# johannes-graeter/mono_lidar_depth

Measured on AMD Instinct MI355X. Metric: feature-depth associations/sec, higher is better.
Workload: dtype f64; 1 GPU; BASELINE config 2: 64x2048 cloud x 2000 features/frame, C0 parameters, 1024 HBM-resident frames/step/GPU; frame_slots_per_launch=1024, features_per_frame=2000, points_per_frame=131072, contexts=2, sequences=1, parallelism=sequence-per-gpu x1

## Files before the change

mono_lidar_depth_amd/csrc/mld_api.hip:

```cpp
#include <hip/hip_runtime.h>

#include <algorithm>

#include <cmath>
#include <cstdio>
#include <cstdlib>
#include <condition_variable>
#include <cstring>
#include <ctime>
#include <functional>
#include <limits>
#include <mutex>
#include <string>
#include <thread>
#include <vector>

#include "../../include/mld.h"
#include "mld_device.h"
#include "mld_kernels.hip"
#include "mld_ransac.hip"

using namespace mld;

namespace {
// ... 31 lines not shown

struct TimedLaunch {
    hipEvent_t e0, e1;
    int which;
};

}

struct FrameHelper {
    std::thread th;
    std::mutex m;
    std::condition_variable cv;
    std::function<int(std::string&)> job;
    bool pending = false, quit = false;
    int rc = 0;
    std::string err;
    void run() {
        std::unique_lock<std::mutex> lk(m);
        for (;;) {
            cv.wait(lk, [&] { return pending || quit; });
            if (quit) return;
            std::function<int(std::string&)> j = std::move(job);
            lk.unlock();
            std::string e;
            const int r = j(e);
            lk.lock();
            rc = r;
            err = std::move(e);
            pending = false;
            cv.notify_all();
        }
    }
    void submit(std::function<int(std::string&)> j) {
        {
            std::lock_guard<std::mutex> lk(m);
            job = std::move(j);
            pending = true;
        }
        cv.notify_all();
    }
    int wait(std::string& e) {
        std::unique_lock<std::mutex> lk(m);
        cv.wait(lk, [&] { return !pending; });
        e = err;
        return rc;
    }
    void stop() {
        {
            std::lock_guard<std::mutex> lk(m);
            quit = true;
        }
        cv.notify_all();
        if (th.joinable()) th.join();
    }
};

struct ProjShare {
    hipStream_t stream = nullptr;
    int refs = 0;
};

struct mld_ctx {
    mld_params P{};
    mld_camera cam{};
    Calib calib{};
    int device = 0;
    hipStream_t stream = nullptr;
    bool own_stream = true;
    std::vector<Slot> slots;
    SlotDesc* d_slots = nullptr;
    unsigned char* dummy = nullptr;
    int32_t* queue_counts = nullptr;
    uint32_t* map_slab = nullptr;
    size_t map_stride = 0;
    int32_t* queue_slab = nullptr;
    uint32_t* bitmaps = nullptr;
    size_t bitmap_words = 0;
    std::vector<SlotDesc> h_descs;
    std::vector<SlotDesc> desc_stage;
    size_t lds_bytes = 0;
    size_t lds_fused = 0;
    size_t lds_classify = 0;
    bool classify_staged = true;
    int bm_ncol = 0, bm_ncolp = 0;
    bool force_thread_path = false;
    size_t proj_lds = 0;
    std::string err;
    int32_t* rs_flags = nullptr;
    int32_t* rs_cand = nullptr;
    int32_t* rs_block = nullptr;
    size_t rs_cap = 0;
    int32_t* rs_M = nullptr;
    int32_t* rs_S = nullptr;
    int32_t* rs_sample = nullptr;
    float* rs_sp = nullptr;
    int32_t* rs_counts = nullptr;
    size_t rs_counts_cap = 0;
    int32_t* rs_inl = nullptr;
    ransac::Result* rs_res = nullptr;
    unsigned char* sem_img = nullptr;
    size_t sem_img_cap = 0;
    float* sem_coeffs = nullptr;
    unsigned char* sem_groups = nullptr;
    size_t sem_groups_cap = 0;
    ransac::SemResult* sem_res = nullptr;
    double* trk_uv_cur = nullptr;
    double* trk_uv_last = nullptr;
    double* trk_depth_cur = nullptr;
    double* trk_depth_last = nullptr;
    int32_t* trk_type_cur = nullptr;
    int32_t* trk_type_last = nullptr;
    int32_t* trk_rank = nullptr;
    long long* trk_n_new = nullptr;
    size_t trk_cap = 0;
    unsigned char* trkb = nullptr;
    size_t trkb_cap = 0;
    int trkb_seqs = 0;
    TrkSeq* trkb_desc = nullptr;
    std::vector<TrkSeq> trkb_host;
    SlotDesc* d_sub = nullptr;
    int32_t* sub_counts = nullptr;
    size_t sub_cap = 0;
    std::vector<SlotDesc> h_sub;
    unsigned char* trk_stage = nullptr;
    size_t trk_stage_cap = 0;
    unsigned char* fr_host = nullptr;
    unsigned char* fr_dev = nullptr;
    size_t fr_cap = 0;
    unsigned char* fr_host_dev = nullptr;
    bool fr_zero_copy = true;
    bool fr_helper_on = true;
    hipEvent_t fr_ev[5] = {nullptr, nullptr, nullptr, nullptr, nullptr};
    double fr_us[10] = {0, 0, 0, 0, 0, 0, 0, 0, 0, 0};
    uint32_t* rsb_masks = nullptr;
    size_t rsb_mask_words = 0;
    PlaneDev* rsb_planes = nullptr;
    uint32_t* rsb_seeds = nullptr;
    hipStream_t side = nullptr;
    hipEvent_t side_done = nullptr, side_start = nullptr;
    FrameHelper* helper = nullptr;
    hipEvent_t order_ev = nullptr;
    mld_ctx* release_waiter = nullptr;
    mld_ctx* waiting_on = nullptr;
    bool order_wait_pending = false;
    uint32_t* cls_done = nullptr;
    uint32_t cls_target = 0;
    const uint32_t* gate_counter = nullptr;
    uint32_t gate_target = 0;
    bool gate_mode = true;
    Calib* d_calib = nullptr;
    Calib calib_uploaded[2]{};
    mld_ctx* gate_src = nullptr;
    mld_ctx* gate_waiter = nullptr;
    hipStream_t proj_stream = nullptr;
    struct ProjShare* proj_share = nullptr;
    hipEvent_t proj_fork = nullptr, proj_join = nullptr;
    size_t lds_fused_pad = 0;
    int queue_probe_tries = 0;
    int queue_shared_with_live = 0;
    int shared_arg = 0;
    int fused_blocks_per_cu = 8;
    size_t lds_per_cu = 0;
    bool timing = false;
    std::vector<TimedLaunch> timed;
    std::vector<hipEvent_t> event_pool;
    static constexpr int kUpGens = 16;
// ... 124 lines not shown
            for (int k = 0; k < 3; k++) {
                ri += (long double)c.Tinv[4 * i + k] * (long double)T[4 * k + 3];
                mi += fabsl((long double)c.Tinv[4 * i + k]) * fabsl((long double)T[4 * k + 3]);
            }
            lin = std::max(lin, rl);
            mlin = std::max(mlin, ml);
            cst = std::max(cst, fabsl(ri));
            mcst = std::max(mcst, mi);
        }
        const long double u64 = 1.1102230246251565e-16L;
        const long double el = lin + 64.0L * u64 * mlin, ec = cst + 64.0L * u64 * mcst;
        const float inf = std::numeric_limits<float>::infinity();
        c.far_elin = (std::isfinite((double)el) && el < 1e30L) ? (float)((double)el * 1.000001) : inf;
        c.far_econst = (std::isfinite((double)ec) && ec < 1e30L) ? (float)((double)ec * 1.000001) : inf;
        if (!(c.far_elin > 0.f)) c.far_elin = 1e-37f;
    }
    c.W = ctx->cam.width;
    c.H = ctx->cam.height;
    c.bmStride = (ctx->cam.height + 16 + 3) / 4 * 4;
    c.halfX1 = (double)P.pixelarea_search_witdh * 0.5 * (double)1.0f;
    c.halfY1 = (double)P.pixelarea_search_height * 0.5 * (double)1.0f;
    c.halfX2 = (double)P.pixelarea_search_witdh * 0.5 * (double)2.0f;
    c.halfY2 = (double)P.pixelarea_search_height * 0.5 * (double)1.5f;
    int cap = window_cells(c.halfX1, c.halfY1);
    if (P.do_use_ransac_plane) cap = std::max(cap, window_cells(c.halfX2, c.halfY2));
    cap = (cap + 1) & ~1;
    c.cap = cap;
    c.binW = P.histogram_segmentation_bin_witdh;
    c.minCount = P.histogram_segmentation_min_pointcount;
    c.countMin = (unsigned)P.radiusSearch_count_min;
    c.useHist = P.do_use_histogram_segmentation;
    c.thrG_en = P.treshold_depth_enabled;
    c.thrG_mode = P.treshold_depth_mode;
    c.thrG_min = (double)P.treshold_depth_min;
    c.thrG_max = (double)P.treshold_depth_max;
    c.thrL_en = P.treshold_depth_local_enabled;
    c.thrL_mode = P.treshold_depth_local_mode;
    c.thrL_type = P.treshold_depth_local_valuetype;
    c.thrL_val = P.treshold_depth_local_value;
    c.useTriMax = P.do_use_triangle_size_maximation;
    c.checkPlanar = P.do_check_triangleplanar_condition;
    c.planarThr = P.triangleplanar_crossnorm_treshold;
    c.orthThr = P.viewray_plane_orthoganality_treshold;
    c.cutBehind = P.do_use_cut_behind_camera;
    c.useRoad = P.do_use_ransac_plane;
    c.roadMode = P.plane_estimator_use_triangle_maximation ? 1 : 0;
    c.roadDistThr = P.ransac_plane_point_distance_treshold;
    c.roadDistThrF = (float)c.roadDistThr;
    c.padf2_ = 0.f;
    c.zxMinRel = P.plane_estimator_z_x_min_relation;
    c.usePCA = P.do_use_PCA;
    c.pcaAbsMin = P.pca_treshold_3_abs_min;
    c.pcaRelMax = P.pca_treshold_3_2_rel_max;
    c.pcaRelMin = P.pca_treshold_2_1_rel_min;
    ctx->lds_bytes = (size_t)cap * (3 * sizeof(double) + 2 * sizeof(int));
    c.threadPath = 1;
    c.xcdAware = 1;
    c.sortClasses = 4;
    c.k1max = 32;
    c.kMain = 24;
    c.kTotal = 40;
#ifdef MLD_AB_SWITCHES
    if (const char* e = std::getenv("MLD_FORCE_WAVE_PATH")) c.threadPath = (e[0] == '1') ? 0 : 1;
    if (const char* e = std::getenv("MLD_NO_XCD")) c.xcdAware = (e[0] == '1') ? 0 : 1;
    if (const char* e = std::getenv("MLD_SORT_CLASSES")) c.sortClasses = (e[0] == '4') ? 4 : 1;
    if (const char* e = std::getenv("MLD_FORCE_THREAD_PATH")) ctx->force_thread_path = e[0] == '1';
    if (const char* e = std::getenv("MLD_PROJ_LDS")) ctx->proj_lds = (size_t)std::atoll(e);
    if (const char* e = std::getenv("MLD_GATE")) ctx->gate_mode = e[0] != '0';
    if (const char* e = std::getenv("MLD_FRAME_COPY")) ctx->fr_zero_copy = e[0] != '1';
    if (const char* e = std::getenv("MLD_FRAME_HELPER")) ctx->fr_helper_on = e[0] != '0';
    if (const char* e = std::getenv("MLD_K1MAX")) c.k1max = std::min(std::max(std::atoi(e), 8), kK1MaxLimit);
    if (const char* e = std::getenv("MLD_KMAIN")) c.kMain = std::min(std::max(std::atoi(e), 8), c.k1max);
    if (std::getenv("MLD_K1MAX") || std::getenv("MLD_KMAIN")) c.kTotal = c.k1max + c.kMain;
    if (const char* e = std::getenv("MLD_KTOTAL")) c.kTotal = std::min(std::max(std::atoi(e), c.k1max), c.k1max + c.kMain);
#endif
    ctx->lds_fused = (size_t)c.kTotal * kWave * sizeof(uint32_t);
    ctx->bm_ncol = (ctx->cam.width + 31) / 32 + 1;
    ctx->bm_ncolp = ctx->bm_ncol | 1;
    const size_t cls_fixed = (size_t)(kClsBuckets + kClsThreads / kWave + 4) * sizeof(int);
    const size_t cls_bitmap = (size_t)c.bmStride * (size_t)ctx->bm_ncolp * sizeof(uint32_t);
    ctx->classify_staged = cls_fixed + cls_bitmap <= 128 * 1024;
#ifdef MLD_AB_SWITCHES
    if (const char* e = std::getenv("MLD_CLASSIFY_STAGED")) ctx->classify_staged = ctx->classify_staged && e[0] != '0';
#endif
    ctx->lds_classify = cls_fixed + (ctx->classify_staged ? cls_bitmap : 0);
}

hipStream_t projection_fork(mld_ctx* ctx, int& rc) {
    rc = MLD_OK;
    if (!ctx->proj_stream) return ctx->stream;
    hipError_t e = hipEventRecord(ctx->proj_fork, ctx->stream);
    if (e == hipSuccess) e = hipStreamWaitEvent(ctx->proj_stream, ctx->proj_fork, 0);
    if (e != hipSuccess) {
        ctx->err = std::string("projection stream (fork): ") + hipGetErrorString(e);
        rc = MLD_ERR_HIP;
    }
    return ctx->proj_stream;
}
int projection_join(mld_ctx* ctx) {
    if (!ctx->proj_stream) return MLD_OK;
    HIP_TRY(ctx, hipEventRecord(ctx->proj_join, ctx->proj_stream));
    HIP_TRY(ctx, hipStreamWaitEvent(ctx->stream, ctx->proj_join, 0));
    return MLD_OK;
}
struct ProjectionScope {
    mld_ctx* ctx;
    bool open = true;
    explicit ProjectionScope(mld_ctx* c) : ctx(c) {}
    int finish() {
        open = false;
        return projection_join(ctx);
    }
    ~ProjectionScope() {
        if (open && ctx->proj_stream) {
            const std::string keep = ctx->err;
            (void)projection_join(ctx);
            ctx->err = keep;
        }
    }
};

int enable_rs_batch_lds(mld_ctx* ctx, size_t lds) {
    static size_t enabled[64] = {};
    static std::mutex mtx;
    std::lock_guard<std::mutex> lk(mtx);
    size_t& cur = enabled[ctx->device & 63];
    if (lds <= cur) return MLD_OK;
    HIP_TRY(ctx, hipFuncSetAttribute(reinterpret_cast<const void*>(ransac::k_rs_batch),
                                     hipFuncAttributeMaxDynamicSharedMemorySize, (int)lds));
    cur = lds;
    return MLD_OK;
}

int check_slot(mld_ctx* ctx, int slot) {
    if (!ctx) return MLD_ERR_INVALID_ARG;
    if (slot < 0 || slot >= (int)ctx->slots.size()) return fail(ctx, MLD_ERR_INVALID_ARG, "slot out of range");
    return MLD_OK;
}

int bind_device(mld_ctx* ctx) {
    HIP_TRY(ctx, hipSetDevice(ctx->device));
    return MLD_OK;
}

template <typename T>
int grow(mld_ctx* ctx, T*& ptr, size_t& cap, size_t need) {
    if (need <= cap && ptr) return MLD_OK;
    if (ptr) {
        HIP_TRY(ctx, hipStreamSynchronize(ctx->stream));
        HIP_TRY(ctx, hipFree(ptr));
        ptr = nullptr;
    }
    size_t n = need < 1 ? 1 : need;
    HIP_TRY(ctx, hipMalloc(reinterpret_cast<void**>(&ptr), n * sizeof(T)));
    cap = n;
    return MLD_OK;
}

hipEvent_t get_event(mld_ctx* ctx) {
    if (!ctx->event_pool.empty()) {
        hipEvent_t e = ctx->event_pool.back();
        ctx->event_pool.pop_back();
        return e;
    }
    hipEvent_t e = nullptr;
    (void)hipEventCreate(&e);
// ... 88 lines not shown
    bool aligned = true;
    for (int i = slot; i < slot + (single ? 1 : n_slots); i++)
        aligned = aligned && (((uintptr_t)ctx->slots[i].d.cloud) & 15) == 0;
    const uint32_t ps_magic = per_slot > 1 ? (uint32_t)(((1ull << 32) + (uint64_t)per_slot - 1) / (uint64_t)per_slot) : 0u;
    if (ctx->order_wait_pending) {
        ctx->order_wait_pending = false;
        if (ctx->gate_counter) {
            hipLaunchKernelGGL(mld::k_gate, dim3(1), dim3(kWave), 0, st, ctx->gate_counter, ctx->gate_target, 100000);
            ctx->gate_counter = nullptr;
            if (ctx->gate_src && ctx->gate_src->gate_waiter == ctx) ctx->gate_src->gate_waiter = nullptr;
            ctx->gate_src = nullptr;
        } else {
            HIP_TRY(ctx, hipStreamWaitEvent(st, ctx->order_ev, 0));
        }
    }
    ScopedTimer tm(ctx, 0, st);
    if (single) {
        auto kp = aligned ? mld::k_project_scatter<true, true> : mld::k_project_scatter<false, true>;
        hipLaunchKernelGGL(kp, dim3(per_slot), dim3(kProjThreads), 0, st, ctx->d_slots, ctx->slots[slot].d, ctx->calib, 1,
                           per_slot, ps_magic, 0u);
    } else {
        auto kp = aligned ? mld::k_project_scatter<true, false> : mld::k_project_scatter<false, false>;
        hipLaunchKernelGGL(kp, dim3((unsigned)per_slot * n_slots), dim3(kProjThreads), ctx->proj_lds, st, ctx->d_slots + slot,
                           SlotDesc{}, ctx->calib, n_slots, per_slot, ps_magic, common_tag(ctx, n_slots, slot));
    }
    HIP_TRY(ctx, hipGetLastError());
    return MLD_OK;
}

int ensure_queues(mld_ctx* ctx, Slot& s, int64_t F) {
    if ((size_t)F <= s.road_cap) return MLD_OK;
    HIP_TRY(ctx, hipStreamSynchronize(ctx->stream));
    if (!s.queues_in_slab) {
        if (s.d.ovf_queue) HIP_TRY(ctx, hipFree(s.d.ovf_queue));
        if (s.d.live_queue) HIP_TRY(ctx, hipFree(s.d.live_queue));
    }
    s.queues_in_slab = false;
    s.d.live_queue = nullptr;
    s.d.ovf_queue = nullptr;
    HIP_TRY(ctx, hipMalloc((void**)&s.d.ovf_queue, (size_t)F * 2 * sizeof(int32_t)));
    HIP_TRY(ctx, hipMalloc((void**)&s.d.live_queue, (size_t)F * sizeof(int32_t)));
    s.road_cap = (size_t)F;
    return MLD_OK;
}

int upload_descs(mld_ctx* ctx, int n_slots, hipStream_t st = nullptr, int first = 0, bool tags_in_descs = false);

int upload_small(mld_ctx* ctx, void* dst, const void* src, size_t bytes, hipStream_t st) {
    static_assert(sizeof(SlotDesc) % 4 == 0 && sizeof(TrkSeq) % 4 == 0 && sizeof(Calib) % 4 == 0, "k_upload moves 32-bit words");
    if (!bytes) return MLD_OK;
    if (bytes % 4) return fail(ctx, MLD_ERR_INVALID_ARG, "upload_small: size not a multiple of 4");
    if (bytes > ctx->up_gen_bytes) return fail(ctx, MLD_ERR_CAPACITY, "upload_small: table larger than the context's upload ring");
    const int g = ctx->up_next;
    if (ctx->up_busy[g]) HIP_TRY(ctx, hipEventSynchronize(ctx->up_ev[g]));
    if (!ctx->up_ev[g]) HIP_TRY(ctx, hipEventCreateWithFlags(&ctx->up_ev[g], hipEventDisableTiming));
    unsigned char* stage = ctx->up_base + (size_t)g * ctx->up_gen_bytes;
    std::memcpy(stage, src, bytes);
    const int words = (int)(bytes / 4);
    hipLaunchKernelGGL(mld::k_upload, dim3((unsigned)((words + 255) / 256)), dim3(256), 0, st, reinterpret_cast<uint32_t*>(dst),
                       reinterpret_cast<const uint32_t*>(stage), words);
    HIP_TRY(ctx, hipGetLastError());
    HIP_TRY(ctx, hipEventRecord(ctx->up_ev[g], st));
    ctx->up_busy[g] = true;
    ctx->up_next = (g + 1) % mld_ctx::kUpGens;
    return MLD_OK;
}

int launch_features(mld_ctx* ctx, int n_slots, int64_t max_F, bool single, int slot, const Calib* override_calib = nullptr,
                    const SlotDesc* group_descs = nullptr) {
    if (max_F <= 0) return MLD_OK;
    const SlotDesc* const descs = group_descs ? group_descs : ctx->d_slots;
    Calib calib = override_calib ? *override_calib : ctx->calib;
    const bool few = single && max_F <= 16384 && !ctx->force_thread_path;
    if (few) calib.threadPath = 0;
    const int per_slot = (int)((max_F + kWave - 1) / kWave);
    const uint32_t tag_all = (single || group_descs) ? 0u : common_tag(ctx, n_slots);
    const SlotDesc one = single ? ctx->slots[slot].d : SlotDesc{};
    const int use_single = single ? 1 : 0, ns = single ? 1 : n_slots;
    if (few) {
    } else {
        ScopedTimer ts(ctx, 5);
        auto kc = ctx->classify_staged ? mld::k_classify<true, kClsThreads, kClsKeep>
                                       : mld::k_classify<false, kClsThreads, kClsKeep>;
        const bool gate = ctx->gate_mode && ctx->release_waiter && !single;
        if (gate && !ctx->cls_done) {
            HIP_TRY(ctx, hipMalloc((void**)&ctx->cls_done, sizeof(uint32_t)));
            HIP_TRY(ctx, hipMemsetAsync(ctx->cls_done, 0, sizeof(uint32_t), ctx->stream));
        }
        hipLaunchKernelGGL(kc, dim3((unsigned)ns), dim3(kClsThreads), ctx->lds_classify, ctx->stream, descs, one,
                           use_single, calib, ctx->bm_ncol, ctx->bm_ncolp, gate ? ctx->cls_done : (uint32_t*)nullptr);
        if (gate) {
            mld_ctx* w = ctx->release_waiter;
            ctx->release_waiter = nullptr;
            w->waiting_on = nullptr;
            ctx->cls_target += (uint32_t)ns;
            if (w->gate_src && w->gate_src != ctx && w->gate_src->gate_waiter == w) w->gate_src->gate_waiter = nullptr;
            if (ctx->gate_waiter && ctx->gate_waiter != w) {
                ctx->gate_waiter->gate_counter = nullptr;
                ctx->gate_waiter->order_wait_pending = false;
                ctx->gate_waiter->gate_src = nullptr;
            }
            w->gate_counter = ctx->cls_done;
            w->gate_target = ctx->cls_target;
            w->order_wait_pending = true;
            w->gate_src = ctx;
            ctx->gate_waiter = w;
        }
    }
    if (ctx->release_waiter) {
        mld_ctx* w = ctx->release_waiter;
        ctx->release_waiter = nullptr;
        w->waiting_on = nullptr;
        HIP_TRY(ctx, hipEventRecord(w->order_ev, ctx->stream));
        if (w->gate_src && w->gate_src->gate_waiter == w) w->gate_src->gate_waiter = nullptr;
        w->gate_src = nullptr;
        w->gate_counter = nullptr;
        w->order_wait_pending = true;
    }
    int rc_up = MLD_OK;
    const Calib* d_calib = ctx->d_calib;
    {
        Calib want = calib;
        want.threadPath = ctx->calib.threadPath;
        const int which = std::memcmp(&want, &ctx->calib, sizeof(Calib)) == 0 ? 0 : 1;
        if (std::memcmp(&want, &ctx->calib_uploaded[which], sizeof(Calib)) != 0) {
            int rc_c = upload_small(ctx, ctx->d_calib + which, &want, sizeof(Calib), ctx->stream);
            if (rc_c) return rc_c;
            ctx->calib_uploaded[which] = want;
        }
        d_calib = ctx->d_calib + which;
    }
    if (calib.threadPath) {
        ScopedTimer tm(ctx, 1);
        int dense = (calib.k1max > 32 || calib.kMain > 24) ? ((ctx->shared_arg & 1) ? 1 : 2) : 0;
#ifdef MLD_AB_SWITCHES
        if (const char* e = std::getenv("MLD_FORCE_DENSE")) dense = std::min(std::max(std::atoi(e), 0), 2);
#endif
        auto kf = dense == 2 ? (calib.roadMode ? mld::k_feature_fused<1, 2> : mld::k_feature_fused<0, 2>)
                  : dense == 1 ? (calib.roadMode ? mld::k_feature_fused<1, 1> : mld::k_feature_fused<0, 1>)
                               : (calib.roadMode ? mld::k_feature_fused<1, 0> : mld::k_feature_fused<0, 0>);
        if (single && (rc_up = upload_descs(ctx, 1, nullptr, slot, true))) return rc_up;
        hipLaunchKernelGGL(kf, dim3((unsigned)per_slot * (unsigned)ns), dim3(kWave), ctx->lds_fused + ctx->lds_fused_pad, ctx->stream,
                           descs + (single ? slot : 0), d_calib, ns, per_slot);
    }
    {
        ScopedTimer tm(ctx, 3);
        const int chunk = few ? (int)std::min<int64_t>(8, std::max<int64_t>(1, (max_F + 8191) / 8192)) : 8;
        const int want = (int)((max_F + chunk - 1) / chunk);
        const int pw = std::max(1, std::min(want, std::max(4, (few ? 16384 : 4096) / ns)));
        auto kw = few ? mld::k_feature_wave<true> : mld::k_feature_wave<false>;
        hipLaunchKernelGGL(kw, dim3((unsigned)pw * (unsigned)ns), dim3(kWave), ctx->lds_bytes, ctx->stream, descs, one,
                           use_single, d_calib, ns, pw, tag_all, chunk);
    }
    HIP_TRY(ctx, hipGetLastError());
    return MLD_OK;
}

int upload_descs(mld_ctx* ctx, int n_slots, hipStream_t st, int first, bool tags_in_descs) {
    if (!st) st = ctx->stream;
    const bool tags_by_arg = !tags_in_descs && common_tag(ctx, n_slots, first) != 0u;
    bool dirty = false;
    ctx->desc_stage.resize((size_t)n_slots);
    for (int i = first; i < first + n_slots; i++) {
        SlotDesc& d = ctx->desc_stage[(size_t)(i - first)];
        d = ctx->slots[i].d;
        if (tags_by_arg) d.tag = 0;
        dirty = dirty || std::memcmp(&d, &ctx->h_descs[i], sizeof(SlotDesc)) != 0;
    }
    if (!dirty) return MLD_OK;
    const int rc = upload_small(ctx, ctx->d_slots + first, ctx->desc_stage.data(), sizeof(SlotDesc) * n_slots, st);
    if (rc != MLD_OK) return rc;
    std::memcpy(ctx->h_descs.data() + first, ctx->desc_stage.data(), sizeof(SlotDesc) * n_slots);
// ... 1810 lines not shown
            }
        }
        if ((rc = upload_small(ctx, ctx->d_sub, ctx->h_sub.data(), n_sub * sizeof(SlotDesc), ctx->stream))) return rc;
        rc = launch_features(ctx, (int)n_sub, Fg, false, 0, nullptr, ctx->d_sub);
    } else {
        if ((rc = upload_descs(ctx, n_desc, nullptr, 0, true))) return rc;
        rc = launch_features(ctx, n_desc, max_n, false, 0);
    }
    for (int q = 0; q < n_seq; q++) ctx->slots[last0 + q].d.F_dev = nullptr;
    if (rc) return rc;
    hipLaunchKernelGGL(k_tracklets_scatter, dim3((unsigned)((max_n + 255) / 256), (unsigned)n_seq), dim3(256), 0, ctx->stream,
                       ctx->trkb_desc);
    HIP_TRY(ctx, hipGetLastError());
    return MLD_OK;
}

int mld_tracklets_depth(mld_ctx* ctx, int slot_cur, int slot_last, const float* u_new, const float* v_new,
                        const float* u_old, const float* v_old, const uint8_t* is_new, int64_t n_tracks,
                        float* d_cur_out, float* d_last_out, int32_t* type_cur_out, int32_t* type_last_out,
                        int64_t* n_new_host) {
    int rc = check_slot(ctx, slot_cur);
    if (rc) return rc;
    if ((rc = bind_device(ctx))) return rc;
    if (n_tracks < 0) return fail(ctx, MLD_ERR_INVALID_ARG, "negative track count");
    if (n_tracks > 0 && (!u_new || !v_new || !u_old || !v_old || !is_new || !d_cur_out || !d_last_out))
        return fail(ctx, MLD_ERR_INVALID_ARG, "null tracklet array");
    const size_t n = (size_t)n_tracks;
    const size_t bytes = n * (4 * 4 + 2 * 4 + 2 * 4 + 1) + 64;
    if ((rc = grow(ctx, ctx->trk_stage, ctx->trk_stage_cap, bytes))) return rc;
    float* du0 = reinterpret_cast<float*>(ctx->trk_stage);
    float *dv0 = du0 + n, *du1 = dv0 + n, *dv1 = du1 + n, *dd0 = dv1 + n, *dd1 = dd0 + n;
    int32_t* dt0 = reinterpret_cast<int32_t*>(dd1 + n);
    int32_t* dt1 = dt0 + n;
    uint8_t* dnew = reinterpret_cast<uint8_t*>(dt1 + n);
    if (n) {
        HIP_TRY(ctx, hipMemcpyAsync(du0, u_new, n * 4, hipMemcpyHostToDevice, ctx->stream));
        HIP_TRY(ctx, hipMemcpyAsync(dv0, v_new, n * 4, hipMemcpyHostToDevice, ctx->stream));
        HIP_TRY(ctx, hipMemcpyAsync(du1, u_old, n * 4, hipMemcpyHostToDevice, ctx->stream));
        HIP_TRY(ctx, hipMemcpyAsync(dv1, v_old, n * 4, hipMemcpyHostToDevice, ctx->stream));
        HIP_TRY(ctx, hipMemcpyAsync(dnew, is_new, n, hipMemcpyHostToDevice, ctx->stream));
        HIP_TRY(ctx, hipMemsetAsync(dd1, 0, n * 4, ctx->stream));
        HIP_TRY(ctx, hipMemsetAsync(dt1, 0, n * 4, ctx->stream));
    }
    rc = mld_tracklets_depth_device(ctx, slot_cur, slot_last, du0, dv0, du1, dv1, dnew, n_tracks, dd0, dd1, dt0, dt1,
                                    nullptr);
    if (rc) return rc;
    if (n) {
        HIP_TRY(ctx, hipMemcpyAsync(d_cur_out, dd0, n * 4, hipMemcpyDeviceToHost, ctx->stream));
        if (type_cur_out) HIP_TRY(ctx, hipMemcpyAsync(type_cur_out, dt0, n * 4, hipMemcpyDeviceToHost, ctx->stream));
        std::vector<float> tmp(n);
        std::vector<int32_t> tmpt(n);
        HIP_TRY(ctx, hipMemcpyAsync(tmp.data(), dd1, n * 4, hipMemcpyDeviceToHost, ctx->stream));
        HIP_TRY(ctx, hipMemcpyAsync(tmpt.data(), dt1, n * 4, hipMemcpyDeviceToHost, ctx->stream));
        HIP_TRY(ctx, hipStreamSynchronize(ctx->stream));
        int64_t nn = 0;
        for (size_t i = 0; i < n; i++)
            if (is_new[i]) {
                d_last_out[i] = tmp[i];
                if (type_last_out) type_last_out[i] = tmpt[i];
                nn++;
            }
        if (n_new_host) *n_new_host = nn;
    } else if (n_new_host) {
        *n_new_host = 0;
    }
    return MLD_OK;
}

int mld_get_path_counts(mld_ctx* ctx, int slot, int64_t* lane_path, int64_t* handed_over) {
    int rc = check_slot(ctx, slot);
    if (rc) return rc;
    if (!lane_path || !handed_over) return fail(ctx, MLD_ERR_INVALID_ARG, "null output");
    if ((rc = bind_device(ctx))) return rc;
    const Slot& s = ctx->slots[slot];
    int32_t live = 0, ovf = 0;
    HIP_TRY(ctx, hipStreamSynchronize(ctx->stream));
    if (s.d.live_count) HIP_TRY(ctx, hipMemcpy(&live, s.d.live_count, sizeof(int32_t), hipMemcpyDeviceToHost));
    if (s.d.ovf_count) HIP_TRY(ctx, hipMemcpy(&ovf, s.d.ovf_count, sizeof(int32_t), hipMemcpyDeviceToHost));
    *lane_path = live;
    *handed_over = ovf;
    return MLD_OK;
}

int mld_get_visible_count(mld_ctx* ctx, int slot, int64_t* n_visible) {
    int rc = check_slot(ctx, slot);
    if (rc) return rc;
    if (!n_visible) return fail(ctx, MLD_ERR_INVALID_ARG, "null output");
    if ((rc = bind_device(ctx))) return rc;
    if ((rc = ensure_full(ctx, ctx->slots[slot]))) return rc;
    *n_visible = ctx->slots[slot].nvis;
    return MLD_OK;
}

int mld_get_visible_image_points(mld_ctx* ctx, int slot, double* uv_out, int64_t capacity) {
    int rc = check_slot(ctx, slot);
    if (rc) return rc;
    if ((rc = bind_device(ctx))) return rc;
    Slot& s = ctx->slots[slot];
    if ((rc = ensure_full(ctx, s))) return rc;
    if (capacity < s.nvis) return fail(ctx, MLD_ERR_CAPACITY, "output buffer too small");
    if (s.nvis) {
        HIP_TRY(ctx, hipMemcpyAsync(uv_out, s.img_vis, (size_t)s.nvis * 2 * sizeof(double), hipMemcpyDeviceToHost, ctx->stream));
        HIP_TRY(ctx, hipStreamSynchronize(ctx->stream));
    }
    return MLD_OK;
}

int mld_get_point_index(mld_ctx* ctx, int slot, int32_t* index_out, int64_t capacity) {
    int rc = check_slot(ctx, slot);
    if (rc) return rc;
    if ((rc = bind_device(ctx))) return rc;
    Slot& s = ctx->slots[slot];
    if ((rc = ensure_full(ctx, s))) return rc;
    if (capacity < s.nvis) return fail(ctx, MLD_ERR_CAPACITY, "output buffer too small");
    if (s.nvis) {
        HIP_TRY(ctx, hipMemcpyAsync(index_out, s.pidx, (size_t)s.nvis * sizeof(int32_t), hipMemcpyDeviceToHost, ctx->stream));
        HIP_TRY(ctx, hipStreamSynchronize(ctx->stream));
    }
    return MLD_OK;
}

int mld_get_cloud_camera_cs(mld_ctx* ctx, int slot, double* xyz_out, int64_t capacity) {
    int rc = check_slot(ctx, slot);
    if (rc) return rc;
    if ((rc = bind_device(ctx))) return rc;
    Slot& s = ctx->slots[slot];
    if ((rc = ensure_full(ctx, s))) return rc;
    if (capacity < s.d.n) return fail(ctx, MLD_ERR_CAPACITY, "output buffer too small");
    if (s.d.n) {
        HIP_TRY(ctx, hipMemcpyAsync(xyz_out, s.cam, (size_t)s.d.n * 3 * sizeof(double), hipMemcpyDeviceToHost, ctx->stream));
        HIP_TRY(ctx, hipStreamSynchronize(ctx->stream));
    }
    return MLD_OK;
}

int mld_get_pixel_map(mld_ctx* ctx, int slot, int32_t* map_out, int64_t capacity) {
    int rc = check_slot(ctx, slot);
    if (rc) return rc;
    if ((rc = bind_device(ctx))) return rc;
    Slot& s = ctx->slots[slot];
    if ((rc = ensure_full(ctx, s))) return rc;
    long long cells = (long long)ctx->cam.width * ctx->cam.height;
    if (capacity < cells) return fail(ctx, MLD_ERR_CAPACITY, "output buffer too small");
    int32_t* tmp = nullptr;
    HIP_TRY(ctx, hipMalloc((void**)&tmp, (size_t)cells * sizeof(int32_t)));
    hipLaunchKernelGGL(k_export_map, dim3((unsigned)((cells + 255) / 256)), dim3(256), 0, ctx->stream, s.d.map, s.d.tag,
                       s.rank, cells, tmp);
    hipError_t e = hipMemcpyAsync(map_out, tmp, (size_t)cells * sizeof(int32_t), hipMemcpyDeviceToHost, ctx->stream);
    if (e == hipSuccess) e = hipStreamSynchronize(ctx->stream);
    (void)hipFree(tmp);
    HIP_TRY(ctx, e);
    return MLD_OK;
}

int mld_get_point_depth_cam_visible(mld_ctx* ctx, int slot, int64_t visible_index, double* depth_out) {
    int rc = check_slot(ctx, slot);
    if (rc) return rc;
    if ((rc = bind_device(ctx))) return rc;
    Slot& s = ctx->slots[slot];
    if ((rc = ensure_full(ctx, s))) return rc;
    if (!depth_out || visible_index < 0 || visible_index >= s.nvis) return fail(ctx, MLD_ERR_INVALID_ARG, "index out of range");
    int32_t raw = 0;
    HIP_TRY(ctx, hipMemcpy(&raw, s.pidx + visible_index, sizeof(int32_t), hipMemcpyDeviceToHost));
    HIP_TRY(ctx, hipMemcpy(depth_out, s.cam + 3 * (size_t)raw + 2, sizeof(double), hipMemcpyDeviceToHost));
    return MLD_OK;
}
// ... 40 lines not shown
```

mono_lidar_depth_amd/csrc/mld_kernels.hip:

```cpp
#include "mld_device.h"
#include "../../include/mld.h"
#include "mld_diag.h"

namespace mld {

#define GPTR(T, p) ((const T __attribute__((address_space(1)))*)(p))
#define GPTRW(T, p) ((T __attribute__((address_space(1)))*)(p))
#define CPTR(T, p) ((const T __attribute__((address_space(4)))*)(p))
typedef float f32x4 __attribute__((ext_vector_type(4)));
typedef uint32_t u32x4u __attribute__((ext_vector_type(4), aligned(4)));

__device__ __forceinline__ int prefix_count(unsigned long long m) {
    return (int)__builtin_amdgcn_mbcnt_hi((unsigned)(m >> 32), __builtin_amdgcn_mbcnt_lo((unsigned)m, 0u));
}
__device__ __forceinline__ int uniform(int v) { return __builtin_amdgcn_readfirstlane(v); }
__device__ __forceinline__ bool wave_any(bool p) { return __builtin_amdgcn_ballot_w64(p) != 0ull; }
__device__ __forceinline__ double readlane_f64(double v, int lane) {
    int lo = __double2loint(v), hi = __double2hiint(v);
    lo = __builtin_amdgcn_readlane(lo, lane);
    hi = __builtin_amdgcn_readlane(hi, lane);
    return __hiloint2double(hi, lo);
}
template <int CTRL, int ROW_MASK>
__device__ __forceinline__ int dpp_self(int v) {
// ... 2137 lines not shown
                const auto* bm = GPTR(uint32_t, s.bitmap) + (size_t)(x0 >> 5) * (size_t)c.bmStride;
                const uint32_t sh = (uint32_t)(x0 & 31);
                const uint32_t colmask = (nx >= 32) ? ~0u : ((1u << nx) - 1u);
                int k1 = 0;
                for (int r = 0; r < ny; r++) {
                    const uint32_t lo = bm[y0 + r], hi = bm[c.bmStride + y0 + r];
                    k1 += __popc(__builtin_amdgcn_alignbit(hi, lo, sh) & colmask);
                }
                if ((unsigned)k1 < c.countMin) {
                    GPTRW(double, s.depth)[f] = -1.0;
                    if (s.type) GPTRW(int32_t, s.type)[f] = MLD_RadiusSearchInsufficientPoints;
                    active = false;
                }
            } else if (nx <= 32) {
                if (0u < c.countMin) {
                    GPTRW(double, s.depth)[f] = -1.0;
                    if (s.type) GPTRW(int32_t, s.type)[f] = MLD_RadiusSearchInsufficientPoints;
                    active = false;
                }
            }
        } else if (active) {
            f = (long long)GPTR(int32_t, s.ovf_queue)[2 * (size_t)(e0 + lane)];
            code = GPTR(int32_t, s.ovf_queue)[2 * (size_t)(e0 + lane) + 1];
            const auto* q = GPTR(double, s.uv) + 2 * f;
            myu = q[0];
            myv = q[1];
        }
        int mytype = code < 0 ? (int)MLD_Unspecified : code;
        double mydepth = -1.0;
        const unsigned long long all = __ballot(active);
        const unsigned long long full = __ballot(active && code < 0);
        double corners[9];
        bool has_corners = false;
        ST_BEGIN(1);
        wave_path(c, s, smem, lane, all, myu, myv, mytype, mydepth, full, corners, has_corners ST_PASS);
        if (active) {
            GPTRW(double, s.depth)[f] = mydepth;
            if (s.type) GPTRW(int32_t, s.type)[f] = mytype;
            if (s.corners && has_corners) {
#pragma unroll
                for (int t = 0; t < 9; t++) GPTRW(double, s.corners)[9 * f + t] = corners[t];
            }
        }
        ST_MARK(12);
        ST_END();
    };
    if (DIRECT) {
        if (j * chunk < count) pass(j * chunk);
    } else {
        for (int e0 = j * chunk; e0 < count; e0 += per_slot * chunk) pass(e0);
    }
}


__device__ __forceinline__ bool window_bounds(const Calib& c, double u, double v, double halfX, double halfY, int& x0,
                                              int& y0, int& nx, int& ny) {
    x0 = 0;
    y0 = 0;
    nx = 0;
    ny = 0;
    if (!(isfinite(u) && isfinite(v))) return false;
    double a;
    a = u - halfX;
    const double left = (a < 0.) ? 0. : a;
    a = u + halfX;
    const double right = ((double)(c.W - 1) < a) ? (double)(c.W - 1) : a;
    a = v - halfY;
    const double top = (a < 0.) ? 0. : a;
    a = v + halfY;
    const double bottom = ((double)(c.H - 1) < a) ? (double)(c.H - 1) : a;
    const int xa = (int)left, ya = (int)top, xb = (int)right, yb = (int)bottom;
    const int wx = xb - xa + 1, wy = yb - ya + 1;
    if (wx <= 0 || wy <= 0 || xa < 0 || ya < 0 || xb >= c.W || yb >= c.H) return false;
    x0 = xa;
    y0 = ya;
    nx = wx;
    ny = wy;
    return true;
}

constexpr int kClsThreads = 1024;
constexpr int kClsBuckets = 1024;
constexpr int kClsKeep = 2;
enum : int { CLS_DEAD = -1, CLS_OVF = -2, CLS_NONE = -3 };

template <bool STAGED, int kClsThreads, int kClsKeep>
__global__ __launch_bounds__(kClsThreads) void k_classify(const SlotDesc* __restrict__ slots, SlotDesc single,
                                                          int use_single, Calib c, int ncol, int ncolp,
                                                          uint32_t* __restrict__ done) {
    extern __shared__ __align__(16) unsigned char smem[];
    int* hist = reinterpret_cast<int*>(smem);
    int* wsum = hist + kClsBuckets;
    int* ctr = wsum + kClsThreads / kWave;
    uint32_t* lbm = reinterpret_cast<uint32_t*>(ctr + 4);
    SlotDesc s = use_single ? single : slots[blockIdx.x];
    apply_plane_dev(s);
    long long Fn = s.F;
    if (s.F_dev) {
        long long fd = *GPTR(long long, s.F_dev) - s.F_dev_off;
        fd = fd < 0 ? 0 : fd;
        Fn = fd < Fn ? fd : Fn;
    }
    const int tid = threadIdx.x, lane = tid & (kWave - 1), wave = tid >> 6;
    if (done && tid == 0) __hip_atomic_fetch_add(GPTRW(uint32_t, done), 1u, __ATOMIC_RELAXED, __HIP_MEMORY_SCOPE_AGENT);
    for (int b = tid; b < kClsBuckets; b += kClsThreads) hist[b] = 0;
    if (tid == 0) ctr[0] = 0;
    const auto* bm = GPTR(uint32_t, s.bitmap);
    if (STAGED) {
        const int q4 = c.bmStride >> 2, n4 = ncol * q4;
        const float rq = 1.0f / (float)q4;
        constexpr int kStage = 4;
        for (int g0 = tid; g0 < n4; g0 += kClsThreads * kStage) {
            u32x4u w[kStage];
            int col[kStage], y[kStage];
#pragma unroll
            for (int t = 0; t < kStage; t++) {
                const int g = g0 + t * kClsThreads;
                col[t] = (int)(((float)g + 0.5f) * rq);
                y[t] = (g - col[t] * q4) << 2;
                w[t] = u32x4u{0u, 0u, 0u, 0u};
                if (g < n4) w[t] = *GPTR(u32x4u, bm + (size_t)col[t] * c.bmStride + y[t]);
            }
#pragma unroll
            for (int t = 0; t < kStage; t++) {
                if (g0 + t * kClsThreads < n4) {
                    lbm[(y[t] + 0) * ncolp + col[t]] = w[t][0];
                    lbm[(y[t] + 1) * ncolp + col[t]] = w[t][1];
                    lbm[(y[t] + 2) * ncolp + col[t]] = w[t][2];
                    lbm[(y[t] + 3) * ncolp + col[t]] = w[t][3];
                }
            }
        }
    }
    __syncthreads();
    const bool road_on = c.useRoad && s.has_plane && s.inlier_mask;
    const auto* uv = GPTR(double, s.uv);
    const int rowBuckets = c.sortClasses > 1 ? kClsBuckets / 4 : kClsBuckets;
    const double scale = (double)rowBuckets / (double)c.H;
    auto count_window = [&](int x0, int y0, int nx, int ny) -> int {
        const int cx = x0 >> 5, sh = x0 & 31;
        const uint32_t colmask = (nx >= 32) ? ~0u : ((1u << nx) - 1u);
        int k = 0;
        if (STAGED) {
            for (int r = 0; r < ny; r++) {
                const int y = y0 + r;
                const uint32_t lo = lbm[y * ncolp + cx], hi = lbm[y * ncolp + cx + 1];
                k += __popc(__builtin_amdgcn_alignbit(hi, lo, (uint32_t)sh) & colmask);
            }
        } else {
            const auto* c0 = bm + (size_t)cx * c.bmStride + y0;
            const auto* c1 = c0 + c.bmStride;
            for (int r0 = 0; r0 < ny; r0 += 4) {
                const u32x4u a = *GPTR(u32x4u, c0 + r0), b = *GPTR(u32x4u, c1 + r0);
#pragma unroll
                for (int q = 0; q < 4; q++)
                    if (r0 + q < ny) k += __popc(__builtin_amdgcn_alignbit(b[q], a[q], (uint32_t)sh) & colmask);
            }
        }
        return k;
    };
    auto classify = [&](double u, double v) -> int {
        int x0, y0, nx, ny;
        int k1 = 0;
        if (window_bounds(c, u, v, c.halfX1, c.halfY1, x0, y0, nx, ny)) {
            if (nx > 32) return CLS_OVF;
            k1 = count_window(x0, y0, nx, ny);
            if (!c.threadPath)
                return ((unsigned)k1 < c.countMin) ? (int)CLS_DEAD : (int)CLS_OVF;
            if (road_on) {
                int a0, a1, anx, any_;
                if (window_bounds(c, u, v, c.halfX2, c.halfY2, a0, a1, anx, any_) && anx > 32) return CLS_OVF;
            }
            if (k1 > c.kMain || k1 > c.kTotal) return CLS_OVF;
            if (road_on && (3 * k1 > c.k1max || 4 * k1 > c.kTotal)) {
                int a0, a1, anx, any_;
                if (window_bounds(c, u, v, c.halfX2, c.halfY2, a0, a1, anx, any_)) {
                    const int k2 = count_window(a0, a1, anx, any_);
                    if (k2 > c.k1max || k1 + k2 > c.kTotal) return CLS_OVF;
                }
            }
        }
        if ((unsigned)k1 < c.countMin) return CLS_DEAD;
        if (!c.threadPath) return CLS_OVF;
        int b = 0;
        if (v > 0.0) b = (v < (double)c.H) ? (int)(v * scale) : rowBuckets - 1;
        b = b < rowBuckets ? b : rowBuckets - 1;
        const int cls = (k1 <= 8) ? 0 : ((k1 <= 12) ? 1 : ((k1 <= 16) ? 2 : 3));
        return (c.sortClasses > 1 ? (3 - cls) * rowBuckets : 0) + b;
    };
    auto settle = [&](long long i, int cls) {
        if (cls == CLS_DEAD) {
            GPTRW(double, s.depth)[i] = -1.0;
            if (s.type) GPTRW(int32_t, s.type)[i] = MLD_RadiusSearchInsufficientPoints;
        } else if (cls == CLS_OVF) {
            const int pos = atomicAdd(&ctr[0], 1);
            GPTRW(int32_t, s.ovf_queue)[2 * (size_t)pos] = (int32_t)i;
            GPTRW(int32_t, s.ovf_queue)[2 * (size_t)pos + 1] = -1;
        }
    };
    int kept[kClsKeep];
    {
        double fu[kClsKeep], fv[kClsKeep];
#pragma unroll
        for (int q = 0; q < kClsKeep; q++) {
            const long long i = tid + (long long)q * kClsThreads;
            fu[q] = 0.0;
            fv[q] = 0.0;
            if (i < Fn) {
                fu[q] = uv[2 * i];
                fv[q] = uv[2 * i + 1];
            }
        }
#pragma unroll
        for (int q = 0; q < kClsKeep; q++) {
            const long long i = tid + (long long)q * kClsThreads;
            kept[q] = (i < Fn) ? classify(fu[q], fv[q]) : (int)CLS_NONE;
            if (kept[q] >= 0) atomicAdd(&hist[kept[q]], 1);
            if (i < Fn) settle(i, kept[q]);
        }
    }
    for (long long i = tid + (long long)kClsKeep * kClsThreads; i < Fn; i += kClsThreads) {
        const int cls = classify(uv[2 * i], uv[2 * i + 1]);
        if (cls >= 0) atomicAdd(&hist[cls], 1);
        settle(i, cls);
    }
    __syncthreads();
    constexpr int kPer = kClsBuckets / kClsThreads;
    static_assert(kPer >= 1 && kPer * kClsThreads == kClsBuckets, "bucket count must be a multiple of the block size");
    int loc[kPer], sum = 0;
#pragma unroll
    for (int q = 0; q < kPer; q++) {
        loc[q] = hist[tid * kPer + q];
        sum += loc[q];
    }
    int incl = sum;
#pragma unroll
    for (int d = 1; d < kWave; d <<= 1) {
        const int t = __shfl_up(incl, d);
        if (lane >= d) incl += t;
    }
    if (lane == kWave - 1) wsum[wave] = incl;
    __syncthreads();
    int base = incl - sum;
    for (int q = 0; q < wave; q++) base += wsum[q];
    if (tid == kClsThreads - 1) {
        *GPTRW(int32_t, s.live_count) = base + sum;
        *GPTRW(int32_t, s.ovf_count) = ctr[0];
    }
#pragma unroll
    for (int q = 0; q < kPer; q++) {
        hist[tid * kPer + q] = base;
        base += loc[q];
    }
    __syncthreads();
    auto* live = GPTRW(int32_t, s.live_queue);
#pragma unroll
    for (int q = 0; q < kClsKeep; q++)
        if (kept[q] >= 0) live[atomicAdd(&hist[kept[q]], 1)] = (int32_t)(tid + q * kClsThreads);
    for (long long i = tid + (long long)kClsKeep * kClsThreads; i < Fn; i += kClsThreads) {
        const int cls = classify(uv[2 * i], uv[2 * i + 1]);
        if (cls >= 0) live[atomicAdd(&hist[cls], 1)] = (int32_t)i;
    }
}

__global__ __launch_bounds__(kWave) void k_gate(const uint32_t* __restrict__ counter, uint32_t target, int max_polls) {
    if (threadIdx.x != 0) return;
    for (int i = 0; i < max_polls; i++) {
        const uint32_t v = __hip_atomic_load(GPTR(uint32_t, counter), __ATOMIC_RELAXED, __HIP_MEMORY_SCOPE_AGENT);
        if ((int32_t)(v - target) >= 0) break;
        __builtin_amdgcn_s_sleep(32);
    }
}

__global__ __launch_bounds__(kWave) void k_probe_wait(const uint32_t* flag, uint32_t* result, int max_polls) {
    if (threadIdx.x != 0) return;
    uint32_t seen = 2u;
    for (int i = 0; i < max_polls; i++) {
        if (__hip_atomic_load(flag, __ATOMIC_RELAXED, __HIP_MEMORY_SCOPE_SYSTEM) != 0u) {
            seen = 1u;
            break;
        }
        __builtin_amdgcn_s_sleep(32);
    }
    __hip_atomic_store(result, seen, __ATOMIC_RELAXED, __HIP_MEMORY_SCOPE_SYSTEM);
}
__global__ void k_probe_set(uint32_t* flag) {
    if (threadIdx.x == 0 && blockIdx.x == 0) __hip_atomic_store(flag, 1u, __ATOMIC_RELAXED, __HIP_MEMORY_SCOPE_SYSTEM);
}

__global__ __launch_bounds__(256) void k_upload(uint32_t* __restrict__ dst, const uint32_t* __restrict__ src_host, int n_words) {
    const int i = blockIdx.x * 256 + threadIdx.x;
    if (i < n_words) dst[i] = __builtin_nontemporal_load(src_host + i);
}

#ifndef MLD_KEY_BATCH_F
#define MLD_KEY_BATCH_F 8
#endif
constexpr int kKeyBatchF = MLD_KEY_BATCH_F;
#ifndef MLD_DENSE_BATCH_MUL
// ... 463 lines not shown
```

Baseline: 2.889 billion feature-depth associations/s.

## Add light classify kernel variant with unstaged bitmap and batched window loads

Adds a classify variant with 256 threads and 8 features per thread that reads the bitmap from global memory instead of staging it in LDS. It prefetches feature coordinates before the plane setup and issues the window bitmap loads for pairs of features together, so the popcounts are computed from preloaded registers. The aim is to skip the LDS staging cost and per-block serialization and to overlap memory latency. In exchange it uses more registers per thread, and the variant is selected by a shared_arg bit or an env switch. A debug queue-readback API is also added.

```diff
diff --git a/mono_lidar_depth_amd/csrc/mld_api.hip b/mono_lidar_depth_amd/csrc/mld_api.hip
--- a/mono_lidar_depth_amd/csrc/mld_api.hip
+++ b/mono_lidar_depth_amd/csrc/mld_api.hip
@@ -137,6 +137,7 @@
     size_t lds_fused = 0;
     size_t lds_classify = 0;
     bool classify_staged = true;
+    int classify_light = -1;
     int bm_ncol = 0, bm_ncolp = 0;
     bool force_thread_path = false;
     size_t proj_lds = 0;
@@ -427,6 +428,7 @@
     ctx->classify_staged = cls_fixed + cls_bitmap <= 128 * 1024;
 #ifdef MLD_AB_SWITCHES
     if (const char* e = std::getenv("MLD_CLASSIFY_STAGED")) ctx->classify_staged = ctx->classify_staged && e[0] != '0';
+    if (const char* e = std::getenv("MLD_CLASSIFY_LIGHT")) ctx->classify_light = (e[0] == '0') ? 0 : ((e[0] == '1') ? 1 : -1);
 #endif
     ctx->lds_classify = cls_fixed + (ctx->classify_staged ? cls_bitmap : 0);
 }
@@ -681,12 +683,21 @@
         ScopedTimer ts(ctx, 5);
         auto kc = ctx->classify_staged ? mld::k_classify<true, kClsThreads, kClsKeep>
                                        : mld::k_classify<false, kClsThreads, kClsKeep>;
+        int cls_threads = kClsThreads;
+        size_t cls_lds = ctx->lds_classify;
+        const bool light = !single && !group_descs && ns > 1 &&
+                           (ctx->classify_light < 0 ? (ctx->shared_arg & 1) != 0 : ctx->classify_light == 1);
+        if (light) {
+            kc = mld::k_classify<false, kClsLightThreads, kClsLightKeep>;
+            cls_threads = kClsLightThreads;
+            cls_lds = (size_t)(kClsBuckets + kClsLightThreads / kWave + 4) * sizeof(int);
+        }
         const bool gate = ctx->gate_mode && ctx->release_waiter && !single;
         if (gate && !ctx->cls_done) {
             HIP_TRY(ctx, hipMalloc((void**)&ctx->cls_done, sizeof(uint32_t)));
             HIP_TRY(ctx, hipMemsetAsync(ctx->cls_done, 0, sizeof(uint32_t), ctx->stream));
         }
-        hipLaunchKernelGGL(kc, dim3((unsigned)ns), dim3(kClsThreads), ctx->lds_classify, ctx->stream, descs, one,
+        hipLaunchKernelGGL(kc, dim3((unsigned)ns), dim3((unsigned)cls_threads), cls_lds, ctx->stream, descs, one,
                            use_single, calib, ctx->bm_ncol, ctx->bm_ncolp, gate ? ctx->cls_done : (uint32_t*)nullptr);
         if (gate) {
             mld_ctx* w = ctx->release_waiter;
@@ -2663,6 +2674,29 @@
     return MLD_OK;
 }
 
+#ifdef MLD_AB_SWITCHES
+int mld_ab_get_queues(mld_ctx* ctx, int slot, int32_t* live_out, int64_t live_cap, int64_t* n_live, int32_t* ovf_out,
+                      int64_t ovf_cap, int64_t* n_ovf) {
+    int rc = check_slot(ctx, slot);
+    if (rc) return rc;
+    if (!live_out || !ovf_out || !n_live || !n_ovf) return fail(ctx, MLD_ERR_INVALID_ARG, "null output");
+    if ((rc = bind_device(ctx))) return rc;
+    const Slot& s = ctx->slots[slot];
+    int32_t live = 0, ovf = 0;
+    HIP_TRY(ctx, hipStreamSynchronize(ctx->stream));
+    if (s.d.live_count) HIP_TRY(ctx, hipMemcpy(&live, s.d.live_count, sizeof(int32_t), hipMemcpyDeviceToHost));
+    if (s.d.ovf_count) HIP_TRY(ctx, hipMemcpy(&ovf, s.d.ovf_count, sizeof(int32_t), hipMemcpyDeviceToHost));
+    if (live < 0 || ovf < 0 || (size_t)live > s.road_cap || (size_t)ovf > s.road_cap)
+        return fail(ctx, MLD_ERR_CAPACITY, "queue lengths beyond the slot's queues");
+    if (live > live_cap || ovf > ovf_cap) return fail(ctx, MLD_ERR_CAPACITY, "output buffer too small");
+    if (live) HIP_TRY(ctx, hipMemcpy(live_out, s.d.live_queue, (size_t)live * sizeof(int32_t), hipMemcpyDeviceToHost));
+    if (ovf) HIP_TRY(ctx, hipMemcpy(ovf_out, s.d.ovf_queue, (size_t)ovf * 2 * sizeof(int32_t), hipMemcpyDeviceToHost));
+    *n_live = live;
+    *n_ovf = ovf;
+    return MLD_OK;
+}
+#endif
+
 int mld_get_visible_count(mld_ctx* ctx, int slot, int64_t* n_visible) {
     int rc = check_slot(ctx, slot);
     if (rc) return rc;
diff --git a/mono_lidar_depth_amd/csrc/mld_kernels.hip b/mono_lidar_depth_amd/csrc/mld_kernels.hip
--- a/mono_lidar_depth_amd/csrc/mld_kernels.hip
+++ b/mono_lidar_depth_amd/csrc/mld_kernels.hip
@@ -2243,6 +2243,8 @@
 constexpr int kClsThreads = 1024;
 constexpr int kClsBuckets = 1024;
 constexpr int kClsKeep = 2;
+constexpr int kClsLightThreads = 256;
+constexpr int kClsLightKeep = 8;
 enum : int { CLS_DEAD = -1, CLS_OVF = -2, CLS_NONE = -3 };
 
 template <bool STAGED, int kClsThreads, int kClsKeep>
@@ -2255,6 +2257,23 @@
     int* ctr = wsum + kClsThreads / kWave;
     uint32_t* lbm = reinterpret_cast<uint32_t*>(ctr + 4);
     SlotDesc s = use_single ? single : slots[blockIdx.x];
+    const int tid = threadIdx.x, lane = tid & (kWave - 1), wave = tid >> 6;
+    constexpr bool kLight = kClsThreads <= 256;
+    const auto* uv = GPTR(double, s.uv);
+    double fu[kClsKeep], fv[kClsKeep];
+    auto fetch_first = [&](long long limit) {
+#pragma unroll
+        for (int q = 0; q < kClsKeep; q++) {
+            const long long i = tid + (long long)q * kClsThreads;
+            fu[q] = 0.0;
+            fv[q] = 0.0;
+            if (i < limit) {
+                fu[q] = uv[2 * i];
+                fv[q] = uv[2 * i + 1];
+            }
+        }
+    };
+    if (kLight) fetch_first(s.F);
     apply_plane_dev(s);
     long long Fn = s.F;
     if (s.F_dev) {
@@ -2262,7 +2281,6 @@
         fd = fd < 0 ? 0 : fd;
         Fn = fd < Fn ? fd : Fn;
     }
-    const int tid = threadIdx.x, lane = tid & (kWave - 1), wave = tid >> 6;
     if (done && tid == 0) __hip_atomic_fetch_add(GPTRW(uint32_t, done), 1u, __ATOMIC_RELAXED, __HIP_MEMORY_SCOPE_AGENT);
     for (int b = tid; b < kClsBuckets; b += kClsThreads) hist[b] = 0;
     if (tid == 0) ctr[0] = 0;
@@ -2295,7 +2313,6 @@
     }
     __syncthreads();
     const bool road_on = c.useRoad && s.has_plane && s.inlier_mask;
-    const auto* uv = GPTR(double, s.uv);
     const int rowBuckets = c.sortClasses > 1 ? kClsBuckets / 4 : kClsBuckets;
     const double scale = (double)rowBuckets / (double)c.H;
     auto count_window = [&](int x0, int y0, int nx, int ny) -> int {
@@ -2320,12 +2337,12 @@
         }
         return k;
     };
-    auto classify = [&](double u, double v) -> int {
+    auto classify = [&](double u, double v, int k1_known = -1) -> int {
         int x0, y0, nx, ny;
         int k1 = 0;
         if (window_bounds(c, u, v, c.halfX1, c.halfY1, x0, y0, nx, ny)) {
             if (nx > 32) return CLS_OVF;
-            k1 = count_window(x0, y0, nx, ny);
+            k1 = (k1_known >= 0) ? k1_known : count_window(x0, y0, nx, ny);
             if (!c.threadPath)
                 return ((unsigned)k1 < c.countMin) ? (int)CLS_DEAD : (int)CLS_OVF;
             if (road_on) {
@@ -2361,21 +2378,57 @@
     };
     int kept[kClsKeep];
     {
-        double fu[kClsKeep], fv[kClsKeep];
+        if (!kLight) fetch_first(Fn);
+        constexpr int kGroup = kLight ? 2 : 1, kRowGroups = 4;
+        static_assert(kClsKeep % kGroup == 0, "the first pass is cut into groups of kGroup features");
+        int k1pre[kClsKeep];
+#pragma unroll
+        for (int q = 0; q < kClsKeep; q++) k1pre[q] = -1;
+        if (kLight) {
+#pragma unroll
+            for (int q0 = 0; q0 < kClsKeep; q0 += kGroup) {
+                int wx0[kGroup], wnx[kGroup], wny[kGroup];
+                bool ok[kGroup];
+                decltype(bm) col0[kGroup];
+                u32x4u wa[kGroup][kRowGroups], wb[kGroup][kRowGroups];
+#pragma unroll
+                for (int g = 0; g < kGroup; g++) {
+                    int y0;
+                    ok[g] = window_bounds(c, fu[q0 + g], fv[q0 + g], c.halfX1, c.halfY1, wx0[g], y0, wnx[g], wny[g]) &&
+                            wnx[g] <= 32;
+                    col0[g] = bm + (size_t)(wx0[g] >> 5) * c.bmStride + y0;
+#pragma unroll
+                    for (int j = 0; j < kRowGroups; j++) {
+                        const int r0 = (4 * j < wny[g]) ? 4 * j : 0;
+                        wa[g][j] = *GPTR(u32x4u, col0[g] + r0);
+                        wb[g][j] = *GPTR(u32x4u, col0[g] + c.bmStride + r0);
+                    }
+                }
+#pragma unroll
+                for (int g = 0; g < kGroup; g++) {
+                    const int sh = wx0[g] & 31;
+                    const uint32_t colmask = (wnx[g] >= 32) ? ~0u : ((1u << wnx[g]) - 1u);
+                    int k = 0;
+#pragma unroll
+                    for (int j = 0; j < kRowGroups; j++)
+#pragma unroll
+                        for (int t = 0; t < 4; t++)
+                            if (4 * j + t < wny[g])
+                                k += __popc(__builtin_amdgcn_alignbit(wb[g][j][t], wa[g][j][t], (uint32_t)sh) & colmask);
+                    for (int r0 = 4 * kRowGroups; r0 < wny[g]; r0 += 4) {
+                        const u32x4u a = *GPTR(u32x4u, col0[g] + r0), b = *GPTR(u32x4u, col0[g] + c.bmStride + r0);
+#pragma unroll
+                        for (int t = 0; t < 4; t++)
+                            if (r0 + t < wny[g]) k += __popc(__builtin_amdgcn_alignbit(b[t], a[t], (uint32_t)sh) & colmask);
+                    }
+                    if (ok[g]) k1pre[q0 + g] = k;
+                }
+            }
+        }
 #pragma unroll
         for (int q = 0; q < kClsKeep; q++) {
             const long long i = tid + (long long)q * kClsThreads;
-            fu[q] = 0.0;
-            fv[q] = 0.0;
-            if (i < Fn) {
-                fu[q] = uv[2 * i];
-                fv[q] = uv[2 * i + 1];
-            }
-        }
-#pragma unroll
-        for (int q = 0; q < kClsKeep; q++) {
-            const long long i = tid + (long long)q * kClsThreads;
-            kept[q] = (i < Fn) ? classify(fu[q], fv[q]) : (int)CLS_NONE;
+            kept[q] = (i < Fn) ? classify(fu[q], fv[q], k1pre[q]) : (int)CLS_NONE;
             if (kept[q] >= 0) atomicAdd(&hist[kept[q]], 1);
             if (i < Fn) settle(i, kept[q]);
         }
```

New measurement: 2.712 billion feature-depth associations/s (median of 2 runs). 6.1% lower.
